# jordi-adell/mcarray

Measured on AMD Instinct MI355X. Metric: STFT frames/sec, 8-mic GCC-PHAT + SRP-PHAT(361) + delay-and-sum beamform @48kHz/1024-pt, higher is better.
Workload: dtype f32 (SRP operands adaptive); 1 GPU; BASELINE configs[2] geometry (8-mic ULA 0.04 m, 48 kHz, N=1024, hop 512, 361 angles, 1 source, no power floor), 8 arrays x 4096 frames per GPU per step; channel rows padded by 64 floats; arrays_per_gpu=8, frames_per_array=4096, srp_precision=adaptive, parallelism=arrays sharded over 1 GPU(s), all_gather of DOA bins+prob

## Files before the change

mcarray_amd/csrc/api.hip:

```cpp
#include "../../include/mcarray_hip.h"
#include "fft1024c.h"
#include "kernels.h"
#include "knobs.h"
#include "stage.h"

#include <chrono>
#include <cmath>
#include <cstdio>
#include <cstdlib>
#include <cstring>
#include <string>
#include <thread>
#include <vector>

using namespace mca;

namespace {

std::string g_create_error;

struct TimedEvent { int id; hipEvent_t a, b; };

}

// ... 1594 lines not shown

static bool steer_applies(const mca_hip_ctx *c)
{
    return !c->generic && !c->n512 && !c->n2048 && c->N == FFT_N && c->M == 8 && c->ula && c->S == 1 && !c->cfg.use_power_floor && c->merged &&
           (c->prec == MCA_HIP_SRP_ADAPTIVE || c->prec == MCA_HIP_SRP_FP16) && c->cfg.gcc_weighting != MCA_HIP_GCC_NONE;
}

static int steer_pass_frames(const mca_hip_ctx *c, int n_arrays, int n_frames)
{
    const long long cap = ws_max_bytes(c) / ((long long)n_arrays * STEER_ROW * (long long)sizeof(float2));
    return (int)std::max<long long>(1, std::min<long long>(n_frames, cap));
}

static void steer_policy_begin(mca_hip_ctx *c)
{
    const unsigned long long s = c->steer_seq + 1;
    if (!c->h_steer || c->steer_lost || s <= FB_LAG) return;
    const unsigned long long r = s - FB_LAG;
    if (r <= c->steer_seq_seen) return;
    const unsigned long long *slot = c->h_steer + 2 * ((r - 1) % FB_RING);
    const auto t0 = std::chrono::steady_clock::now();
    while (__atomic_load_n(&slot[1], __ATOMIC_ACQUIRE) != r) {
        if (std::chrono::duration_cast<std::chrono::milliseconds>(std::chrono::steady_clock::now() - t0).count() > FB_WAIT_MS) { c->steer_lost = true; c->steer_spec = true; return; }
        std::this_thread::yield();
    }
    c->steer_seq_seen = r;
    c->steer_spec = __atomic_load_n(&slot[0], __ATOMIC_RELAXED) * STEER_MISS_DEN <= c->steer_call_frames[(r - 1) % FB_RING] * STEER_MISS_NUM;
}

static int steer_prepare(mca_hip_ctx *c, int n_arrays, int n_frames)
{
    if (!c->d_steer_rows) {
        const size_t na = (size_t)c->cfg.max_arrays;
        HIP_TRY(c, hipMalloc((void **)&c->d_steer_rows, (size_t)(c->D + 1) * 4 * 64 * sizeof(float4)));
        HIP_TRY(c, hipMalloc((void **)&c->d_steer_q, (size_t)(c->D + 1) * c->M * 8 * sizeof(float2)));
        HIP_TRY(c, hipMalloc((void **)&c->d_steer_nyq, (size_t)(c->D + 1) * c->M * sizeof(float)));
        HIP_TRY(c, hipMalloc((void **)&c->d_steer_pred, na * sizeof(int)));
        HIP_TRY(c, hipMalloc((void **)&c->d_steer_miss, 3 * sizeof(unsigned long long)));
        if (hipHostMalloc((void **)&c->h_steer, FB_RING * 16, hipHostMallocDefault) == hipSuccess) std::memset(c->h_steer, 0, FB_RING * 16); else { c->h_steer = nullptr; (void)hipGetLastError(); }
        HIP_TRY(c, hipMalloc((void **)&c->d_steer_tail, 2 * na * FFT_H * sizeof(float)));
        HIP_TRY(c, hipMemset(c->d_steer_pred, 0xff, na * sizeof(int)));
        HIP_TRY(c, hipMemset(c->d_steer_miss, 0, 3 * sizeof(unsigned long long)));
        const double unit = (double)c->cfg.sample_rate / (double)FFT_N / 346.1;
        hipLaunchKernelGGL(k_steer_table, dim3(c->D + 1, 4), dim3(64), 0, nullptr, c->d_steer_rows, c->d_steer_q, c->d_steer_nyq, c->d_grid, c->d_micx, c->M, unit);
        HIP_TRY(c, hipGetLastError());
        HIP_TRY(c, hipDeviceSynchronize());
    }
    const size_t rows = (size_t)n_arrays * steer_pass_frames(c, n_arrays, n_frames);
    if (rows > c->steer_Y_rows) {
        HIP_TRY(c, hipDeviceSynchronize());
        if (c->d_steer_Y) (void)hipFree(c->d_steer_Y);
        c->d_steer_Y = nullptr; c->steer_Y_rows = 0;
        HIP_TRY(c, hipMalloc((void **)&c->d_steer_Y, rows * STEER_ROW * sizeof(float2)));
        c->steer_Y_rows = rows;
    }
    return MCA_HIP_OK;
}

static int steer_reserve(mca_hip_ctx *c, int n_arrays, int n_frames) { return steer_applies(c) ? steer_prepare(c, n_arrays, n_frames) : MCA_HIP_OK; }

static int steer_separate(mca_hip_ctx *c, const float *pcm, long long array_stride, long long mic_stride, int n_arrays, int n_frames,
                          const int *doa_bin, float *out_pcm, hipStream_t st)
{
    const size_t a0 = (size_t)c->a0;
    const int pf = steer_pass_frames(c, n_arrays, n_frames);
    const bool fused = c->steer_fused_now && pf == n_frames;
    const size_t smem = (size_t)(F1K_TWORDS + 4 * F1K_SCRATCH) * sizeof(float2);
    float *tails[2] = {c->d_steer_tail, c->d_steer_tail + (size_t)c->cfg.max_arrays * FFT_H};
    time_begin(c, MCA_HIP_K_BEAMFORM, st);
    int pass = 0;
    for (int f0 = 0; f0 < n_frames; f0 += pf, ++pass) {
        const int f1 = std::min(n_frames, f0 + pf), np = f1 - f0;
        const bool last = f1 == n_frames;
        SteerPatchArgs pa{};
        pa.pcm = pcm; pa.array_stride = array_stride; pa.mic_stride = mic_stride; pa.n_arrays = n_arrays; pa.n_frames = n_frames; pa.f0 = f0; pa.f1 = f1;
        pa.window = c->d_window; pa.doa_bin = doa_bin; pa.all = fused ? 0 : 1; pa.miss = c->d_steer_miss;
        pa.bf.rows = c->d_steer_rows; pa.bf.q = c->d_steer_q; pa.bf.nyq = c->d_steer_nyq; pa.bf.pred = c->d_steer_pred + a0; pa.bf.Y = c->d_steer_Y;
        pa.y_f0 = f0; pa.y_frames = fused ? n_frames : np;
        hipLaunchKernelGGL(k_steer_patch, dim3(std::min(STEER_PATCH_WGS, (np + 3) / 4)), dim3(256), smem, st, pa);
        SteerSynthArgs sy{};
        sy.Y = c->d_steer_Y; sy.n_frames = n_frames; sy.f0 = f0; sy.f1 = f1; sy.y_f0 = pa.y_f0; sy.y_frames = pa.y_frames;
        sy.ft = 16;
        while (sy.ft > 2 && (long long)n_arrays * ((np + sy.ft - 1) / sy.ft) < 1024) sy.ft >>= 1;
        sy.out = out_pcm;
        sy.tail_in = pass == 0 ? c->d_tail[c->tail_cur] + a0 * FFT_H : tails[(pass - 1) & 1];
        sy.tail_out = last ? c->d_tail[c->tail_cur ^ 1] + a0 * FFT_H : tails[pass & 1];
        sy.doa_bin = doa_bin; sy.pred_out = last ? c->d_steer_pred + a0 : nullptr;
        if (last && c->h_steer) { sy.report = c->h_steer + 2 * (c->steer_seq % FB_RING); sy.seq = c->steer_seq + 1; sy.miss_total = c->d_steer_miss; }
        const int runs = (np + sy.ft - 1) / sy.ft;
        hipLaunchKernelGGL(k_steer_synth, dim3((runs + 3) / 4, n_arrays), dim3(256), smem, st, sy);
    }
    time_end(c, st);
    HIP_TRY(c, hipGetLastError());
    c->steer_call_frames[c->steer_seq % FB_RING] = (unsigned long long)n_arrays * n_frames; ++c->steer_seq;
    c->steer_frames_total += (unsigned long long)n_arrays * n_frames;
    if (fused) ++c->steer_fused_calls;
    return MCA_HIP_OK;
}

static int separate_impl(mca_hip_ctx *c, const float *pcm, long long array_stride, long long mic_stride,
                         int n_arrays, int n_frames, const float *doa_rad, float *out_pcm, hipStream_t st, const int *doa_bin = nullptr)
{
    const size_t a0 = (size_t)c->a0;
    if (doa_bin && c->d_bftab && c->n2048 && (reinterpret_cast<uintptr_t>(out_pcm) & 7) == 0) {
        BeamformWaveArgs wa{};
        wa.pcm = pcm; wa.array_stride = array_stride; wa.mic_stride = mic_stride;
        wa.M = c->M; wa.n_pairs = c->M; wa.n_frames = n_frames; wa.S = c->S;
        wa.ft = 16;
        for (int ft = 2; ft <= 64; ++ft)
            if ((long long)n_arrays * c->S * ((n_frames + 4 * ft - 2) / (4 * ft - 1)) <= 2LL * c->n_cu) { wa.ft = ft; break; }
        wa.window = c->d_window; wa.doa_bin = doa_bin; wa.table = c->d_bftab; wa.out = out_pcm;
        wa.tail_in = c->d_tail[c->tail_cur] + a0 * c->S * c->H; wa.tail_out = c->d_tail[c->tail_cur ^ 1] + a0 * c->S * c->H;
        const int wgs = (n_frames + 4 * wa.ft - 2) / (4 * wa.ft - 1);
        const size_t smem_w = (size_t)(F1K_TWORDS + 4 * F1K_SCRATCH + 4 * 512) * sizeof(float2);
        time_begin(c, MCA_HIP_K_BEAMFORM, st);
        hipLaunchKernelGGL(k_beamform_wave_2048, dim3(wgs, n_arrays, c->S), dim3(256), smem_w, st, wa);
        time_end(c, st);
        HIP_TRY(c, hipGetLastError());
        return MCA_HIP_OK;
    }
    if (doa_bin && c->d_bftab && wave_beamformer_applies(c)) {
        BeamformWaveArgs wa{};
        wa.pcm = pcm; wa.array_stride = array_stride; wa.mic_stride = mic_stride;
        wa.M = c->M; wa.n_pairs = c->bf_pairs; wa.n_frames = n_frames; wa.S = c->S;
        wa.window = c->d_window; wa.doa_bin = doa_bin; wa.table = c->d_bftab; wa.out = out_pcm;
        wa.tail_in = c->d_tail[c->tail_cur] + a0 * c->S * c->H; wa.tail_out = c->d_tail[c->tail_cur ^ 1] + a0 * c->S * c->H;
        if (c->S >= 2 && c->M <= 8) {
            wa.ft = 16;
            while (wa.ft > 2 && (long long)n_arrays * ((n_frames + wa.ft - 1) / wa.ft) < 2048) wa.ft >>= 1;
            const int runs = (n_frames + wa.ft - 1) / wa.ft;
            const size_t smem_ms = (size_t)(F1K_TWORDS + 4 * F1K_SCRATCH) * sizeof(float2) + (size_t)4 * c->S * FFT_H * sizeof(float);
            const dim3 gms((runs + 3) / 4, n_arrays);
            time_begin(c, MCA_HIP_K_BEAMFORM, st);
#define BFMS(NPT)                                                                                                                   \
            do {                                                                                                                    \
                if (smem_ms > 64 * 1024) {                                                                                          \
                    HIP_TRY(c, hipFuncSetAttribute(reinterpret_cast<const void *>(&k_beamform_wave_ms<NPT, false>), hipFuncAttributeMaxDynamicSharedMemorySize, (int)smem_ms)); \
                    HIP_TRY(c, hipFuncSetAttribute(reinterpret_cast<const void *>(&k_beamform_wave_ms<NPT, true>), hipFuncAttributeMaxDynamicSharedMemorySize, (int)smem_ms));  \
                }                                                                                                                   \
                if (c->M & 1) hipLaunchKernelGGL((k_beamform_wave_ms<NPT, true>), gms, dim3(256), smem_ms, st, wa);                 \
                else hipLaunchKernelGGL((k_beamform_wave_ms<NPT, false>), gms, dim3(256), smem_ms, st, wa);                         \
            } while (0)
            if (c->bf_pairs == 1) {
                if (smem_ms > 64 * 1024) HIP_TRY(c, hipFuncSetAttribute(reinterpret_cast<const void *>(&k_beamform_wave_ms<1, false>), hipFuncAttributeMaxDynamicSharedMemorySize, (int)smem_ms));
                hipLaunchKernelGGL((k_beamform_wave_ms<1, false>), gms, dim3(256), smem_ms, st, wa);
            }
            else if (c->bf_pairs == 2) BFMS(2);
            else if (c->bf_pairs == 3) BFMS(3);
            else BFMS(4);
#undef BFMS
            time_end(c, st);
            HIP_TRY(c, hipGetLastError());
            return MCA_HIP_OK;
        }
        wa.ft = 2;
        while (wa.ft < 256 && (long long)n_arrays * c->S * ((n_frames + 4 * wa.ft - 2) / (4 * wa.ft - 1)) > 512) ++wa.ft;
        const int wgs = (n_frames + 4 * wa.ft - 2) / (4 * wa.ft - 1);
        const size_t smem = (size_t)(F1K_TWORDS + 4 * F1K_SCRATCH) * sizeof(float2) + 4 * FFT_H * sizeof(float);
        dim3 gb(wgs, n_arrays, c->S);
        if (c->S == 1 && (wgs & 1) == 0 && wa.ft >= 8 && (long long)wgs * n_arrays > (long long)c->n_cu * 3 / 2 && (long long)wgs * n_arrays <= 2LL * c->n_cu) {
            wa.skew = (3 * wa.ft + 8) / 16;
            if (wa.skew >= wa.ft) wa.skew = 0;
            else gb = dim3(n_arrays, wgs, c->S);
        }
        time_begin(c, MCA_HIP_K_BEAMFORM, st);
        if (c->M & 1) hipLaunchKernelGGL(k_beamform_wave<true>, gb, dim3(256), smem, st, wa);
// ... 956 lines not shown
```

mcarray_amd/csrc/fft1024c.h:

```cpp
#pragma once
#include "fft512.h"

namespace mca {

constexpr int F1K_ROW = 18;
constexpr int F1K_SCRATCH = 64 * F1K_ROW;
constexpr int F1K_TWORDS = 64 * F1K_ROW;

__device__ __forceinline__ void f1k_table_init(float2 *tab, int tid, int nthreads)
{
    for (int e = tid; e < 1024; e += nthreads) tab[(e >> 4) * F1K_ROW + (e & 15)] = twiddle(((e >> 4) * (e & 15)) & 1023, 1024, false);
}

__device__ __forceinline__ float2 csub_jb(float2 a, float2 b)
{
    v2f av = to_v2f(a), bv = to_v2f(b), r;
    asm("v_pk_fma_f32 %0, %2, 1.0, %1 op_sel:[1,0,0] op_sel_hi:[0,0,1] neg_hi:[1,0,0]" : "=v"(r) : "v"(av), "v"(bv));
    return from_v2f(r);
}
__device__ __forceinline__ float2 cadd_jb(float2 a, float2 b)
{
    v2f av = to_v2f(a), bv = to_v2f(b), r;
    asm("v_pk_fma_f32 %0, %2, 1.0, %1 op_sel:[1,0,0] op_sel_hi:[0,0,1] neg_lo:[1,0,0]" : "=v"(r) : "v"(av), "v"(bv));
    return from_v2f(r);
}
__device__ __forceinline__ float2 cscale(float2 a, float s)
{
    v2f av = to_v2f(a), sv = {s, s}, r;
    asm("v_pk_mul_f32 %0, %1, %2" : "=v"(r) : "v"(av), "v"(sv));
    return from_v2f(r);
}
__device__ __forceinline__ float2 cmul_mj(float2 a)
{
    v2f av = to_v2f(a), one = {1.f, 1.f}, r;
    asm("v_pk_mul_f32 %0, %1, %2 op_sel:[1,0] op_sel_hi:[0,1] neg_hi:[1,0]" : "=v"(r) : "v"(av), "v"(one));
    return from_v2f(r);
}
__device__ __forceinline__ float2 cmul_pj(float2 a)
{
    v2f av = to_v2f(a), one = {1.f, 1.f}, r;
    asm("v_pk_mul_f32 %0, %1, %2 op_sel:[1,0] op_sel_hi:[0,1] neg_lo:[1,0]" : "=v"(r) : "v"(av), "v"(one));
    return from_v2f(r);
}

template <bool INV>
__device__ __forceinline__ void bfly4(float2 &a0, float2 &a1, float2 &a2, float2 &a3)
{
    const float2 t0 = cadd(a0, a2), t1 = csub(a0, a2), t2 = cadd(a1, a3), t3 = csub(a1, a3);
    a0 = cadd(t0, t2);
    a2 = csub(t0, t2);
    if (!INV) { a1 = csub_jb(t1, t3); a3 = cadd_jb(t1, t3); }
    else { a1 = cadd_jb(t1, t3); a3 = csub_jb(t1, t3); }
}

__device__ __forceinline__ constexpr int dr16(int p) { return (p >> 2) + 4 * (p & 3); }

template <bool INV>
__device__ __forceinline__ void fft16(float2 (&v)[16])
{
    constexpr float R = 0.70710678118654752440f, C1 = 0.92387953251128675613f, S1 = 0.38268343236508977173f;
#pragma unroll
    for (int j = 0; j < 4; ++j) bfly4<INV>(v[j], v[j + 4], v[j + 8], v[j + 12]);
    const float2 w1 = make_float2(C1, -S1), w3 = make_float2(S1, -C1), w9 = make_float2(-C1, S1);
    if (!INV) {
        v[5] = cmul(v[5], w1);  v[9] = cscale(csub_jb(v[9], v[9]), R);   v[13] = cmul(v[13], w3);
        v[6] = cscale(csub_jb(v[6], v[6]), R);  v[10] = cmul_mj(v[10]);   v[14] = cscale(cadd_jb(v[14], v[14]), -R);
        v[7] = cmul(v[7], w3);  v[11] = cscale(cadd_jb(v[11], v[11]), -R); v[15] = cmul(v[15], w9);
    } else {
        v[5] = cmulc(v[5], w1); v[9] = cscale(cadd_jb(v[9], v[9]), R);   v[13] = cmulc(v[13], w3);
        v[6] = cscale(cadd_jb(v[6], v[6]), R);  v[10] = cmul_pj(v[10]);   v[14] = cscale(csub_jb(v[14], v[14]), -R);
        v[7] = cmulc(v[7], w3); v[11] = cscale(csub_jb(v[11], v[11]), -R); v[15] = cmulc(v[15], w9);
    }
#pragma unroll
    for (int q = 0; q < 4; ++q) bfly4<INV>(v[4 * q], v[4 * q + 1], v[4 * q + 2], v[4 * q + 3]);
}

__device__ __forceinline__ void lds_read16_b128(float2 (&v)[16], const float2 *p)
{
    typedef float v4f __attribute__((ext_vector_type(4)));
    v4f a[8];
    asm volatile(
        "ds_read_b128 %0, %8\n\tds_read_b128 %1, %8 offset:16\n\tds_read_b128 %2, %8 offset:32\n\tds_read_b128 %3, %8 offset:48\n\t"
        "ds_read_b128 %4, %8 offset:64\n\tds_read_b128 %5, %8 offset:80\n\tds_read_b128 %6, %8 offset:96\n\tds_read_b128 %7, %8 offset:112\n\t"
        "s_waitcnt lgkmcnt(0)"
        : "=&v"(a[0]), "=&v"(a[1]), "=&v"(a[2]), "=&v"(a[3]), "=&v"(a[4]), "=&v"(a[5]), "=&v"(a[6]), "=&v"(a[7])
        : "v"((unsigned)(uintptr_t)p)
        : "memory");
#pragma unroll
    for (int i = 0; i < 8; ++i) { v[2 * i] = make_float2(a[i].x, a[i].y); v[2 * i + 1] = make_float2(a[i].z, a[i].w); }
}

__device__ __forceinline__ void swap_rows32(float &a, float &b)
{
    const auto r = __builtin_amdgcn_permlane32_swap(__float_as_uint(a), __float_as_uint(b), false, false);
    a = __uint_as_float(r[0]); b = __uint_as_float(r[1]);
}
__device__ __forceinline__ void swap_rows16(float &a, float &b)
{
    const auto r = __builtin_amdgcn_permlane16_swap(__float_as_uint(a), __float_as_uint(b), false, false);
    a = __uint_as_float(r[0]); b = __uint_as_float(r[1]);
}
__device__ __forceinline__ void transpose_rows4(float2 &x0, float2 &x1, float2 &x2, float2 &x3)
{
    swap_rows32(x0.x, x2.x); swap_rows32(x0.y, x2.y); swap_rows32(x1.x, x3.x); swap_rows32(x1.y, x3.y);
    swap_rows16(x0.x, x1.x); swap_rows16(x0.y, x1.y); swap_rows16(x2.x, x3.x); swap_rows16(x2.y, x3.y);
}

struct F1kNoMid { __device__ __forceinline__ void operator()() const {} };

struct F1kLane {
    float2 wb[4];
    float2 t1[16];
    __device__ __forceinline__ void init(int lane)
    {
#pragma unroll
        for (int q = 1; q < 4; ++q) wb[q] = twiddle(((lane & 15) * q) & 63, 64, false);
    }
    __device__ __forceinline__ void load_t1(const float2 *tab, int lane)
    {
#pragma unroll
        for (int q = 0; q < 16; ++q) t1[q] = tab[lane * 18 + q];
    }
};

template <bool INV, int OPT = 3, typename Mid = F1kNoMid>
__device__ __forceinline__ void fft1024c(float2 (&v)[16], float2 *buf, int lane, const float2 *tab, const F1kLane &lc, Mid mid = Mid(), int row = -1)
{
    constexpr bool SCHED = OPT & 2, T1REG = OPT & 4;
    float2 tw[16];
    if (!T1REG) {
        lds_read16_b128(tw, tab + lane * F1K_ROW);
        if (SCHED) __builtin_amdgcn_sched_barrier(0);
    }
    fft16<INV>(v);
#pragma unroll
    for (int p = 1; p < 16; ++p) {
        const float2 w = T1REG ? lc.t1[dr16(p)] : tw[dr16(p)];
        v[p] = INV ? cmulc(v[p], w) : cmul(v[p], w);
    }
#pragma unroll
    for (int q = 0; q < 4; ++q) transpose_rows4(v[4 * q], v[4 * q + 1], v[4 * q + 2], v[4 * q + 3]);
#pragma unroll
    for (int q = 0; q < 4; ++q) bfly4<INV>(v[4 * q], v[4 * q + 1], v[4 * q + 2], v[4 * q + 3]);
    float2 *wr = buf + (lane >> 4) * (4 * F1K_ROW) + (lane & 15);
#pragma unroll
    for (int q = 0; q < 4; ++q)
#pragma unroll
        for (int kb = 0; kb < 4; ++kb) {
            if (kb != 0) v[4 * q + kb] = INV ? cmulc(v[4 * q + kb], lc.wb[kb]) : cmul(v[4 * q + kb], lc.wb[kb]);
            wr[(q + 16 * kb) * F1K_ROW] = v[4 * q + kb];
        }
    wave_lds_fence();
    mid();
    if (SCHED) __builtin_amdgcn_sched_barrier(0);
    lds_read16_b128(v, buf + (row < 0 ? lane : row) * F1K_ROW);
    wave_lds_fence();
    fft16<INV>(v);
}

}
```

mcarray_amd/csrc/kernels_wave.hip:

```cpp
#include <type_traits>

#include "fft1024c.h"
#include "mca_internal.h"
#include "cand_unit.h"
#include "phat_pairs.h"
#include "pair_balance.h"
#include "steer.h"

namespace mca {

__global__ __launch_bounds__(256) void k_bf_table(float2 *tab, const float *grid, const double *mic_x, int M, int n_pairs, double unit)
{
    const int d = blockIdx.x, pr = blockIdx.y;
    const double doa = d == 0 ? 0.0 : (double)grid[d - 1];
    const double cd = cos(doa + 1.57079632679489661923);
    const double sc = 1.0 / ((double)M * 1024.0);
    float2 *row = tab + ((long long)d * n_pairs + pr) * 1024;
    for (int k = threadIdx.x; k < 1024; k += 256) {
        const int kap = k <= 512 ? k : k - 1024;
        double pa[2] = {0.0, 0.0}, pb[2] = {0.0, 0.0};
        for (int e = 0; e < 2; ++e) {
            const int c = 2 * pr + e;
            if (c >= M) continue;
            double turns = (double)kap * (unit * mic_x[c] * cd);
// ... 539 lines not shown
                for (int s = 0; s < 8; ++s) {
                    if constexpr (ULA) {
                        float2 r[MT], out[NOUT];
#pragma unroll
                        for (int m = 0; m < MT; ++m) r[m] = Xh[m][s];
                        pair_products<MT, ULA>(r, out);
#pragma unroll
                        for (int g = 0; g < NOUT; ++g) store_a_wave<PL2>(arow, voff, g * KG + 64 * s, out[g], p.Kp);
                    } else {
                        int pi = 0;
#pragma unroll
                        for (int i = 0; i < MT; ++i)
#pragma unroll
                            for (int j = i + 1; j < MT; ++j) { store_a_wave<PL2>(arow, voff, pi * KG + 64 * s, cmulc(Xh[i][s], Xh[j][s]), p.Kp); ++pi; }
                    }
                }
            }
            if (POWER) {
                const float pacc = wave_sum64(ptime.x + ptime.y);
                if (lane == 0) p.power[(long long)a * p.total_frames + p.frame0 + f] = pacc / (float)FFT_N / (float)MT;
            }
        }
        wave_lds_fence();
        if (!MERGE && lane < f_end - f_begin) {
            float2 xn[MT], out[NOUT];
#pragma unroll
            for (int pr = 0; pr < NP; ++pr) {
                const float2 n = nyq[lane * NP + pr];
                float pw;
                xn[2 * pr] = whiten4<NOPHAT>(make_float2(2.f * n.x, 0.f), pw);
                xn[2 * pr + 1] = whiten4<NOPHAT>(make_float2(2.f * n.y, 0.f), pw);
            }
            OutT *arow = reinterpret_cast<OutT *>(p.A) + (row_base + f_begin + lane) * (long long)p.a_row_elems;
            pair_products<MT, ULA>(xn, out);
#pragma unroll
            for (int g = 0; g < NOUT; ++g) store_a_wave<PL2>(arow, 0u, g * KG + FFT_H, out[g], p.Kp);
        }
        }
        wave_lds_fence();
        if constexpr (CAND) {
            static_assert(!CAND || PL2, "the candidate contraction reads the two-plane rows of the list mode");
            {
                __syncthreads();
                cand_unit<4>(p.cand, li - p.list0, e_unit, reinterpret_cast<unsigned char *>(wbase), tid);
            }
        }
    }
}

__global__ __launch_bounds__(64) void k_steer_table(float4 *rows, float2 *q, float *nyq, const float *grid, const double *mic_x, int M, double unit)
{
    const int d = blockIdx.x, pr = blockIdx.y, lane = threadIdx.x, lam = lane <= 32 ? lane : 96 - lane;
    const double doa = d == 0 ? 0.0 : (double)grid[d - 1];
    const double cd = cos(doa + 1.57079632679489661923);
    const double sc = 1.0 / ((double)M * 1024.0);
    auto phasor = [&](int c, int k, double &cs, double &sn) {
        double turns = (double)k * (unit * mic_x[c] * cd);
        turns -= rint(turns);
        sincospi(2.0 * turns, &sn, &cs);
    };
    double ca, sa, cb, sb;
    phasor(2 * pr, lam, ca, sa); phasor(2 * pr + 1, lam, cb, sb);
    rows[((long long)d * gridDim.y + pr) * 64 + lane] = make_float4((float)(ca * sc), (float)(sa * sc), (float)(cb * sc), (float)(sb * sc));
    if (lane < 16) {
        const int c = 2 * pr + (lane >> 3), s = lane & 7;
        double cs, sn;
        phasor(c, 64 * s, cs, sn);
        q[((long long)d * M + c) * 8 + s] = make_float2((float)cs, (float)sn);
    }
    if (lane < 2) {
        double cs, sn;
        phasor(2 * pr + lane, 512, cs, sn);
        nyq[d * M + 2 * pr + lane] = (float)(cs * sc);
    }
}

__global__ __launch_bounds__(256, 2) void k_steer_patch(SteerPatchArgs p)
{
    constexpr int NP = 4, MT = 8;
    extern __shared__ __attribute__((aligned(16))) unsigned char smem_raw[];
    float2 *tab = reinterpret_cast<float2 *>(smem_raw);
    const int tid = threadIdx.x, lane = tid & 63, wave = __builtin_amdgcn_readfirstlane(tid >> 6);
    float2 *buf = tab + F1K_TWORDS + wave * F1K_SCRATCH;
    const int npass = p.f1 - p.f0, stride = 4 * (int)gridDim.x;
    int work = p.all;
    if (!work) {
        for (int a = 0; a < p.n_arrays; ++a) {
            const int pred = p.bf.pred[a];
            for (int fo = (int)blockIdx.x * 4 + wave + stride * lane; fo < npass; fo += stride * 64)
                work |= p.doa_bin[(long long)a * p.n_frames + p.f0 + fo] != pred;
        }
    }
    if (!__syncthreads_or(work)) return;
    f1k_table_init(tab, tid, 256);
    F1kLane lc;
    lc.init(lane);
    __syncthreads();
    const int lam = lane <= 32 ? lane : 96 - lane;
    const bool self = (lane & 31) == 0;
    v2f win[8];
#pragma unroll
    for (int i = 0; i < 8; ++i) { win[i].x = p.window[lane + 128 * i]; win[i].y = p.window[lane + 128 * i + 64]; }
    for (int a = 0; a < p.n_arrays; ++a) {
        const int pred = __builtin_amdgcn_readfirstlane(p.bf.pred[a]);
        const bool every = p.all != 0;
        int missed = 0;
        for (int fo = (int)blockIdx.x * 4 + wave; fo < npass; fo += stride) {
            const int f = p.f0 + fo;
            const int bin = __builtin_amdgcn_readfirstlane(p.doa_bin[(long long)a * p.n_frames + f]);
            if (bin != pred) ++missed;
            else if (!every) continue;
            const float4 *srow = p.bf.rows + (long long)(bin + 1) * (NP * 64);
            const float2 *qrow = p.bf.q + (long long)(bin + 1) * (MT * 8);
            const float *base = p.pcm + (long long)a * p.array_stride + (long long)f * FFT_H;
            float2 *yrow = p.bf.Y + ((long long)a * p.y_frames + f - p.y_f0) * STEER_ROW;
            float xa[16], xb[16];
            auto load_pair = [&](int pr) {
                const float *pa = base + (long long)(2 * pr) * p.mic_stride, *pb = pa + p.mic_stride;
#pragma unroll
                for (int i = 0; i < 16; ++i) { xa[i] = pa[(unsigned)lane + 64 * i]; xb[i] = pb[(unsigned)lane + 64 * i]; }
            };
            load_pair(0);
            float2 Y[8], zn[NP];
#pragma unroll
            for (int pr = 0; pr < NP; ++pr) {
                float2 z[16];
                float4 B;
#pragma unroll
                for (int i = 0; i < 8; ++i) { z[2 * i] = win_lo(xa[2 * i], xb[2 * i], win[i]); z[2 * i + 1] = win_hi(xa[2 * i + 1], xb[2 * i + 1], win[i]); }
                float ma = max3abs(z[0].x, z[1].x, z[2].x), mb = max3abs(z[0].y, z[1].y, z[2].y);
#pragma unroll
                for (int i = 3; i < 15; i += 2) { ma = max3abs(ma, z[i].x, z[i + 1].x); mb = max3abs(mb, z[i].y, z[i + 1].y); }
                ma = max2abs(ma, z[15].x); mb = max2abs(mb, z[15].y);
                const PairBalance pb = pair_balance(ma, mb);
                if (pb.scaled()) {
                    const float sa = pb.sa(), sb = pb.sb();
#pragma unroll
                    for (int i = 0; i < 16; ++i) z[i] = make_float2(z[i].x * sa, z[i].y * sb);
                }
                fft1024c<false, 3>(z, buf, lane, tab, lc, [&]() {
                    B = (srow + pr * 64)[(unsigned)lane];
                    if (pr < NP - 1) load_pair(pr + 1);
                }, lam);
                const float un_a = pb.un_a(), un_b = pb.un_b();
                zn[pr] = make_float2(z[dr16(8)].x * un_a, z[dr16(8)].y * un_b);
                const float4 Bu = steer_base(B, un_a, un_b);
                if (lane == 0) {
                    float2 t[16];
#pragma unroll
                    for (int j = 0; j < 16; ++j) t[j] = z[dr16(j)];
#pragma unroll
                    for (int j = 8; j < 16; ++j) z[dr16(j < 12 ? j + 4 : j - 4)] = t[(j + 1) & 15];
                } else if (self) {
#pragma unroll
                    for (int j = 8; j < 12; ++j) { const float2 t = z[dr16(j)]; z[dr16(j)] = z[dr16(j + 4)]; z[dr16(j + 4)] = t; }
                } else {
#pragma unroll
                    for (int j = 8; j < 12; ++j) {
                        float2 &u = z[dr16(j)], &w = z[dr16(j + 4)];
                        swap_rows32(u.x, w.x); swap_rows32(w.x, u.x);
                        swap_rows32(u.y, w.y); swap_rows32(w.y, u.y);
                    }
                }
#pragma unroll
                for (int s = 0; s < 8; ++s) {
                    const float2 zk = z[dr16(s)], zm = z[dr16(15 - s < 12 ? 15 - s + 4 : 15 - s - 4)];
                    const float2 a2 = make_float2(zk.x + zm.x, zk.y - zm.y);
                    const float2 b2 = make_float2(zk.y + zm.y, zm.x - zk.x);
                    const float2 y = pr == 0 ? make_float2(0.f, 0.f) : Y[s];
                    if (s == 0) Y[s] = steer_mac<true>(y, a2, b2, Bu, a2, b2);
                    else Y[s] = steer_mac<false>(y, a2, b2, Bu, qrow[(2 * pr) * 8 + s], qrow[(2 * pr + 1) * 8 + s]);
                }
                wave_lds_fence();
            }
#pragma unroll
            for (int s = 0; s < 8; ++s) yrow[(unsigned)lam + 64 * s] = s == 0 ? steer_dc(Y[s], lane) : Y[s];
            if (lane == 0) yrow[FFT_H] = make_float2(steer_nyquist<NP>(zn, p.bf.nyq + (bin + 1) * MT), 0.f);
        }
        if (missed && lane == 0) { atomicAdd(p.miss, (unsigned long long)missed); if (pred >= 0) atomicAdd(p.miss + 1, (unsigned long long)missed); }
    }
}

__global__ __launch_bounds__(256) void k_steer_synth(SteerSynthArgs p)
{
    extern __shared__ __attribute__((aligned(16))) unsigned char smem_raw[];
    float2 *tab = reinterpret_cast<float2 *>(smem_raw);
    const int tid = threadIdx.x, lane = tid & 63, wave = __builtin_amdgcn_readfirstlane(tid >> 6);
    float2 *buf = tab + F1K_TWORDS + wave * F1K_SCRATCH;
    f1k_table_init(tab, tid, 256);
    F1kLane lc;
    lc.init(lane);
    __syncthreads();
    const int a = blockIdx.y;
    if (p.pred_out && blockIdx.x == 0 && tid == 0) p.pred_out[a] = p.doa_bin[(long long)a * p.n_frames + p.n_frames - 1];
    if (p.report && blockIdx.x == 0 && a == 0 && tid == 0) {
        const unsigned long long tot = p.miss_total[1];
        p.report[0] = tot - p.miss_total[2];
        p.miss_total[2] = tot;
        __hip_atomic_store(&p.report[1], p.seq, __ATOMIC_RELEASE, __HIP_MEMORY_SCOPE_SYSTEM);
    }
    const int t0 = p.f0 + ((int)blockIdx.x * 4 + wave) * p.ft, t1 = min(t0 + p.ft, p.f1);
    if (t0 >= t1) return;
    const float2 *Yb = p.Y + ((long long)a * p.y_frames - p.y_f0) * STEER_ROW;
    float *ob = p.out + (long long)a * p.n_frames * FFT_H;
    float carry[8];
    if (t0 == p.f0) {
#pragma unroll
        for (int i = 0; i < 8; ++i) carry[i] = p.tail_in[(long long)a * FFT_H + lane + 64 * i];
    }
    int t = t0 > p.f0 ? t0 - 1 : t0;
    float2 yv[8], nv[8];
    float yn, nn = 0.f;
#pragma unroll
    for (int i = 0; i < 8; ++i) yv[i] = Yb[(long long)t * STEER_ROW + (unsigned)lane + 64 * i];
    yn = Yb[(long long)t * STEER_ROW + FFT_H].x;
    for (; t < t1; ++t) {
        float2 y[16];
        steer_inverse(y, yv, yn, buf, lane, tab, lc, [&]() {
            if (t + 1 < t1) {
#pragma unroll
                for (int i = 0; i < 8; ++i) nv[i] = Yb[(long long)(t + 1) * STEER_ROW + (unsigned)lane + 64 * i];
                nn = Yb[(long long)(t + 1) * STEER_ROW + FFT_H].x;
            }
        });
        if (t >= t0) {
#pragma unroll
            for (int i = 0; i < 8; ++i) ob[(long long)t * FFT_H + (unsigned)lane + 64 * i] = carry[i] + y[dr16(i)].x;
        }
#pragma unroll
        for (int i = 0; i < 8; ++i) { carry[i] = y[dr16(i + 8)].x; yv[i] = nv[i]; }
        yn = nn;
    }
    if (t1 == p.f1) {
#pragma unroll
        for (int i = 0; i < 8; ++i) p.tail_out[(long long)a * FFT_H + lane + 64 * i] = carry[i];
    }
}

typedef _Float16 h2 __attribute__((ext_vector_type(2)));
__device__ __forceinline__ h2 rot_j_conj(h2 b)
{
    h2 r;
    const unsigned c = 0x3C00BC00u;
    asm("v_pk_mul_f16 %0, %1, %2 op_sel:[1,0] op_sel_hi:[0,1]" : "=v"(r) : "v"(b), "v"(c));
    return r;
}

template <bool POWER>
__global__ __launch_bounds__(256, 2) void k_stft_phat_wave16(StftPhatArgs p)
{
    constexpr int MT = 16, NP = 8;
    extern __shared__ __attribute__((aligned(16))) unsigned char smem_raw[];
    float2 *tab = reinterpret_cast<float2 *>(smem_raw);
    const int tid = threadIdx.x, lane = tid & 63, wave = __builtin_amdgcn_readfirstlane(tid >> 6);
    float2 *buf = tab + F1K_TWORDS + wave * F1K_SCRATCH;
    float *wtab = reinterpret_cast<float *>(tab + F1K_TWORDS + 4 * F1K_SCRATCH);
    const int fpa = p.fpb + p.skew;
    float2 *nyq = reinterpret_cast<float2 *>(wtab + 1024) + wave * (fpa * NP);
    float2 *nref = reinterpret_cast<float2 *>(wtab + 1024) + 4 * (fpa * NP) + wave * (fpa * NP);
    float *dcbad = reinterpret_cast<float *>(reinterpret_cast<float2 *>(wtab + 1024) + 8 * (fpa * NP)) + wave * fpa;
    constexpr float UNSURE = 1e-10f;
    for (int e = tid; e < 1024; e += 256) wtab[(e & 63) * 16 + (e >> 6)] = p.window[e];
    f1k_table_init(tab, tid, 256);
    F1kLane lc;
    lc.init(lane);
    __syncthreads();
    const int lam = lane <= 32 ? lane : 96 - lane;
    const unsigned voff = (unsigned)lam * 4u;
    const bool self = (lane & 31) == 0;
    const float4 *wq = reinterpret_cast<const float4 *>(wtab + lane * 16);

    const int a = p.skew ? blockIdx.x : blockIdx.y;
    int f_begin = ((int)blockIdx.x * 4 + wave) * p.fpb, f_end = min(f_begin + p.fpb, p.n_frames);
    if (p.skew) {
        const int g = blockIdx.y, half = gridDim.y >> 1, hi = p.fpb + p.skew, lo = p.fpb - p.skew;
        if (g < half) { f_begin = (g * 4 + wave) * hi; f_end = f_begin + hi; }
        else { f_begin = half * 4 * hi + ((g - half) * 4 + wave) * lo; f_end = f_begin + lo; }
    }
    if (f_begin >= f_end) return;
    const long long row_base = (long long)a * p.n_frames;
    const float *base = p.pcm + (long long)a * p.array_stride + lane;
    float xa[16], xb[16];
    auto load_pair = [&](int f, int pr) {
        const float *pa = base + (long long)(2 * pr) * p.mic_stride + (long long)(p.frame0 + f) * FFT_H;
        const float *pb = pa + p.mic_stride;
#pragma unroll
        for (int i = 0; i < 16; ++i) { xa[i] = pa[64 * i]; xb[i] = pb[64 * i]; }
    };
    const int nfr = f_end - f_begin;
    const int rot = (int)((unsigned)(5 * a + 3 * ((int)blockIdx.x * 4 + wave)) % (unsigned)nfr);
    auto frame_of = [&](int i) { const int j = i + rot; return f_begin + (j >= nfr ? j - nfr : j); };
    load_pair(frame_of(0), 0);
    for (int fi = 0; fi < nfr; ++fi) {
        const int f = frame_of(fi);
        h2 Xh[MT][8];
        v2f ptime = {0.f, 0.f};
        bool dc_unsure = false;
#pragma unroll
        for (int pr = 0; pr < NP; ++pr) {
            float2 z[16];
#pragma unroll
            for (int i4 = 0; i4 < 4; ++i4) {
                const float4 w4 = wq[i4];
                const v2f w01 = {w4.x, w4.y}, w23 = {w4.z, w4.w};
                z[4 * i4] = win_lo(xa[4 * i4], xb[4 * i4], w01); z[4 * i4 + 1] = win_hi(xa[4 * i4 + 1], xb[4 * i4 + 1], w01);
                z[4 * i4 + 2] = win_lo(xa[4 * i4 + 2], xb[4 * i4 + 2], w23); z[4 * i4 + 3] = win_hi(xa[4 * i4 + 3], xb[4 * i4 + 3], w23);
            }
            float ref_a = 0.f, ref_b = 0.f;
            if (POWER || p.unsure) {
                v2f pz = {0.f, 0.f};
#pragma unroll
                for (int i = 0; i < 16; ++i) { const v2f zv = to_v2f(z[i]); asm("v_pk_fma_f32 %0, %1, %1, %0" : "+v"(pz) : "v"(zv)); }
                if (POWER) { ptime.x += pz.x; ptime.y += pz.y; }
                if (p.unsure) { ref_a = 4.f * wave_sum64(pz.x); ref_b = 4.f * wave_sum64(pz.y); }
// ... 127 lines not shown
```

mcarray_amd/csrc/mca_internal.h:

```cpp
#pragma once
#include <hip/hip_runtime.h>

#define MCA_MAX_SOURCES 4
#define MCA_MAX_MICS 16

namespace mca {

constexpr int MK_NB = 4;
constexpr int MK_WARM = 8;
constexpr int BF_NB = 4;
constexpr int GCC2_DOAWARM = 64;
constexpr int SCAN_WARM = 96;
constexpr int KG = 513;
#ifndef MCA_SCAN_CHUNK
#define MCA_SCAN_CHUNK 32
#endif
#ifndef MCA_SCAN_SUB
#define MCA_SCAN_SUB 32
#endif
constexpr int SCAN_CHUNK = MCA_SCAN_CHUNK;
constexpr int SCAN_SUB = MCA_SCAN_SUB;
#ifndef MCA_SCAN_LD
#define MCA_SCAN_LD 8
#endif
constexpr int SCAN_LD = MCA_SCAN_LD;
#ifndef MCA_REPAIR_WARM
#define MCA_REPAIR_WARM 16
#endif
constexpr int REPAIR_WARM = MCA_REPAIR_WARM;
constexpr int REPAIR_GROUP = 4;
constexpr int HIST_FRAMES = REPAIR_WARM, HIST_UNITS = HIST_FRAMES / REPAIR_GROUP, HIST_SAMPLES = (HIST_FRAMES + 1) * 512;
static_assert(HIST_FRAMES % REPAIR_GROUP == 0, "history = whole repair units");

constexpr int CAND_WORDS_MAX = 20;
struct CandArgs {
    const void *A;
    const void *B;
    int Kp, Dp, a_row_elems;
    const int *list; const int *n_list; int list0, pass_rows;
    unsigned *umask; int umask_words;
    int *need;
    int groups_per_array, n_frames;
    float *C; int c_planes; long long c_plane_stride;
    float *hist_C; int hist_base;
};

constexpr int STEER_QWORDS = 8 * 7;
constexpr int STEER_LDS_ROWS = 13;
constexpr int STEER_Y_ZN = 8, STEER_Y_BASE = 11;
constexpr int STEER_MISS_NUM = 1, STEER_MISS_DEN = 3;
constexpr int STEER_ROW = 520;
struct SteerArgs {
    const float4 *rows;
    const float2 *q;
    const float *nyq;
    const int *pred;
    float2 *Y;
};
constexpr int STEER_PATCH_WGS = 512;
struct SteerPatchArgs {
    const float *pcm; long long array_stride, mic_stride;
    int n_arrays, n_frames;
    int f0, f1;
    const float *window;
    const int *doa_bin;
    SteerArgs bf;
    int y_f0, y_frames;
    int all;
    unsigned long long *miss;
};
struct SteerSynthArgs {
    const float2 *Y; int n_frames, f0, f1, ft, y_f0, y_frames;
    float *out;
    const float *tail_in; float *tail_out;
    const int *doa_bin; int *pred_out;
    unsigned long long *report; unsigned long long seq; unsigned long long *miss_total;
};

struct StftPhatArgs {
    const float *pcm;
    long long array_stride, mic_stride;
    int M, n_frames, frame0, fpb;
    const float *window;
    void *A;
    int Kp;
    int a_row_elems;
    int a_planes;
    float *power;
    int total_frames;
    int N, logH, kg, ula;
    const float2 *tw;
    const int *list; const int *n_list; int list0, list_cap, groups_per_array;
    float *hist_out; const float *hist_in; int hist_base;
    const unsigned short *mrank; int n_merged;
    int no_phat;
    int skew;
    unsigned char *dead;
    unsigned char *unsure;
    int cand_on; CandArgs cand;
    SteerArgs bf;
};

__device__ __forceinline__ void store_a(float *row, const StftPhatArgs &, int cidx, float2 v)
{
    reinterpret_cast<float2 *>(row)[cidx] = v;
}

typedef _Float16 half2_t __attribute__((ext_vector_type(2)));

typedef float float2_t __attribute__((ext_vector_type(2)));

__device__ __forceinline__ void store_a(_Float16 *row, const StftPhatArgs &p, int cidx, float2 v)
{
    const float2_t vv = {v.x, v.y};
    const half2_t hi = __builtin_convertvector(vv, half2_t);
    reinterpret_cast<half2_t *>(row)[cidx] = hi;
    if (p.a_planes == 2) {
        const float2_t back = __builtin_convertvector(hi, float2_t);
        const half2_t lo = __builtin_convertvector(vv - back, half2_t);
        reinterpret_cast<half2_t *>(row + p.Kp)[cidx] = lo;
    }
}

struct GemmArgs {
    const void *A;
    const void *B;
    float *C;
    int rows;
    int chunk_frames, total_frames, frame0;
    int Kp, Dp, a_row_elems;
    long long c_plane_elems;
    const void *Bt;
    const int *n_list; int list0;
    int repair_ksplit;
    int repair_items;
    float *part; int *nvoiced; int D, n_chunks;
    long long part_plane_stride;
    float scan_w[32];
};

struct ScanPickArgs {
    const float *C;
    int c_planes; long long c_plane_stride;
    int n_frames, Dp, D, P, S, chunk, n_chunks;
    float mu, one_minus_mu;
    float inv_norm;
    const float *state_in;
    float *state_out;
    float *part;
    int part_planes; long long part_plane_stride;
    int *nvoiced;
    float *e_start;
    const unsigned char *voiced;
    const float *grid;
    int *doa_bin; float *doa_rad; float *prob; float *energy;
// ... 378 lines not shown
```

mcarray_amd/csrc/steer.h:

```cpp
#pragma once
#include "fft1024c.h"

namespace mca {

__device__ __forceinline__ float4 steer_base(float4 B, float un_a, float un_b)
{
    const float2 a = cscale(make_float2(B.x, B.y), un_a), b = cscale(make_float2(B.z, B.w), un_b);
    return make_float4(a.x, a.y, b.x, b.y);
}
template <bool FIRST>
__device__ __forceinline__ float2 steer_mac(float2 y, float2 a2, float2 b2, float4 B, float2 qa, float2 qb)
{
    if (!FIRST) { a2 = cmul(a2, qa); b2 = cmul(b2, qb); }
    y = cmac(y, a2, make_float2(B.x, B.y));
    return cmac(y, b2, make_float2(B.z, B.w));
}
__device__ __forceinline__ float2 steer_dc(float2 y0, int lane) { return cscale(y0, lane == 0 ? 0.5f : 1.f); }

template <int NP>
__device__ __forceinline__ float steer_nyquist(const float2 (&zn)[NP], const float *pn)
{
    float yn = 0.f;
#pragma unroll
    for (int pr = 0; pr < NP; ++pr) yn = fmaf(zn[pr].y, pn[2 * pr + 1], fmaf(zn[pr].x, pn[2 * pr], yn));
    return yn;
}

template <typename Mid = F1kNoMid>
__device__ __forceinline__ void steer_inverse(float2 (&y)[16], const float2 (&yv)[8], float yn, float2 *buf, int lane, const float2 *tab, const F1kLane &lc, Mid mid = Mid())
{
#pragma unroll
    for (int i = 0; i < 8; ++i) { y[i] = yv[i]; y[i + 8] = make_float2(0.f, 0.f); }
    fft1024c<true, 3>(y, buf, lane, tab, lc, mid);
    const float sn = (lane & 1) ? -yn : yn;
#pragma unroll
    for (int i = 0; i < 16; ++i) y[i].x += sn;
}

}
```

Baseline: 57.47 million frames/s.

## Restructure steer patch/synth: slot-ballot scheduling, warmup handoff, and half-zero inverse FFT

Steer patch now flattens (array, frame) pairs into slots, evaluates DOA misses via wave ballots, and processes only missed slots. It also prefetches the first PCM pair and window before table init, and accumulates miss counters per block. Steer synth adds an LDS handoff between waves so non-lead waves skip recomputing the previous frame's inverse FFT for overlap-add, and the inverse FFT uses a specialized first radix-16 stage that exploits the zero upper half. This adds a block barrier and more complex indexing, with a risk of ordering bugs in the handoff.

```diff
diff --git a/mcarray_amd/csrc/api.hip b/mcarray_amd/csrc/api.hip
--- a/mcarray_amd/csrc/api.hip
+++ b/mcarray_amd/csrc/api.hip
@@ -1700,6 +1700,7 @@
         sy.Y = c->d_steer_Y; sy.n_frames = n_frames; sy.f0 = f0; sy.f1 = f1; sy.y_f0 = pa.y_f0; sy.y_frames = pa.y_frames;
         sy.ft = 16;
         while (sy.ft > 2 && (long long)n_arrays * ((np + sy.ft - 1) / sy.ft) < 1024) sy.ft >>= 1;
+        sy.handoff = sy.ft == 16;
         sy.out = out_pcm;
         sy.tail_in = pass == 0 ? c->d_tail[c->tail_cur] + a0 * FFT_H : tails[(pass - 1) & 1];
         sy.tail_out = last ? c->d_tail[c->tail_cur ^ 1] + a0 * FFT_H : tails[pass & 1];
diff --git a/mcarray_amd/csrc/fft1024c.h b/mcarray_amd/csrc/fft1024c.h
--- a/mcarray_amd/csrc/fft1024c.h
+++ b/mcarray_amd/csrc/fft1024c.h
@@ -75,6 +75,23 @@
     for (int q = 0; q < 4; ++q) bfly4<INV>(v[4 * q], v[4 * q + 1], v[4 * q + 2], v[4 * q + 3]);
 }
 
+__device__ __forceinline__ void fft16_inv_lo8(float2 (&v)[16])
+{
+    constexpr float R = 0.70710678118654752440f, C1 = 0.92387953251128675613f, S1 = 0.38268343236508977173f;
+#pragma unroll
+    for (int j = 0; j < 4; ++j) {
+        const float2 a0 = v[j], a1 = v[j + 4];
+        v[j] = cadd(a0, a1); v[j + 8] = csub(a0, a1);
+        v[j + 4] = cadd_jb(a0, a1); v[j + 12] = csub_jb(a0, a1);
+    }
+    const float2 w1 = make_float2(C1, -S1), w3 = make_float2(S1, -C1), w9 = make_float2(-C1, S1);
+    v[5] = cmulc(v[5], w1); v[9] = cscale(cadd_jb(v[9], v[9]), R);   v[13] = cmulc(v[13], w3);
+    v[6] = cscale(cadd_jb(v[6], v[6]), R);  v[10] = cmul_pj(v[10]);   v[14] = cscale(csub_jb(v[14], v[14]), -R);
+    v[7] = cmulc(v[7], w3); v[11] = cscale(csub_jb(v[11], v[11]), -R); v[15] = cmulc(v[15], w9);
+#pragma unroll
+    for (int q = 0; q < 4; ++q) bfly4<true>(v[4 * q], v[4 * q + 1], v[4 * q + 2], v[4 * q + 3]);
+}
+
 __device__ __forceinline__ void lds_read16_b128(float2 (&v)[16], const float2 *p)
 {
     typedef float v4f __attribute__((ext_vector_type(4)));
@@ -158,4 +175,33 @@
     fft16<INV>(v);
 }
 
-}
+template <typename Mid = F1kNoMid>
+__device__ __forceinline__ void fft1024c_inv_lo8(float2 (&v)[16], float2 *buf, int lane, const float2 *tab, const F1kLane &lc, Mid mid = Mid())
+{
+    float2 tw[16];
+    lds_read16_b128(tw, tab + lane * F1K_ROW);
+    __builtin_amdgcn_sched_barrier(0);
+    fft16_inv_lo8(v);
+#pragma unroll
+    for (int p = 1; p < 16; ++p) v[p] = cmulc(v[p], tw[dr16(p)]);
+#pragma unroll
+    for (int q = 0; q < 4; ++q) transpose_rows4(v[4 * q], v[4 * q + 1], v[4 * q + 2], v[4 * q + 3]);
+#pragma unroll
+    for (int q = 0; q < 4; ++q) bfly4<true>(v[4 * q], v[4 * q + 1], v[4 * q + 2], v[4 * q + 3]);
+    float2 *wr = buf + (lane >> 4) * (4 * F1K_ROW) + (lane & 15);
+#pragma unroll
+    for (int q = 0; q < 4; ++q)
+#pragma unroll
+        for (int kb = 0; kb < 4; ++kb) {
+            if (kb != 0) v[4 * q + kb] = cmulc(v[4 * q + kb], lc.wb[kb]);
+            wr[(q + 16 * kb) * F1K_ROW] = v[4 * q + kb];
+        }
+    wave_lds_fence();
+    mid();
+    __builtin_amdgcn_sched_barrier(0);
+    lds_read16_b128(v, buf + lane * F1K_ROW);
+    wave_lds_fence();
+    fft16<true>(v);
+}
+
+}
diff --git a/mcarray_amd/csrc/kernels_wave.hip b/mcarray_amd/csrc/kernels_wave.hip
--- a/mcarray_amd/csrc/kernels_wave.hip
+++ b/mcarray_amd/csrc/kernels_wave.hip
@@ -645,45 +645,73 @@
     float2 *tab = reinterpret_cast<float2 *>(smem_raw);
     const int tid = threadIdx.x, lane = tid & 63, wave = __builtin_amdgcn_readfirstlane(tid >> 6);
     float2 *buf = tab + F1K_TWORDS + wave * F1K_SCRATCH;
-    const int npass = p.f1 - p.f0, stride = 4 * (int)gridDim.x;
-    int work = p.all;
-    if (!work) {
-        for (int a = 0; a < p.n_arrays; ++a) {
-            const int pred = p.bf.pred[a];
-            for (int fo = (int)blockIdx.x * 4 + wave + stride * lane; fo < npass; fo += stride * 64)
-                work |= p.doa_bin[(long long)a * p.n_frames + p.f0 + fo] != pred;
-        }
-    }
-    if (!__syncthreads_or(work)) return;
+    const int npass = p.f1 - p.f0, stride = 4 * (int)gridDim.x, first = (int)blockIdx.x * 4 + wave;
+    const int nown = first < npass ? (npass - 1 - first) / stride + 1 : 0, nslot = nown * p.n_arrays;
+    const unsigned ndiv = (unsigned)max(nown, 1);
+    struct Slot { int pred, bin; bool in; };
+    auto ask = [&](int s0) {
+        const unsigned s = (unsigned)(s0 + lane), q = s / ndiv;
+        Slot r;
+        r.in = (int)s < nslot;
+        const unsigned a = r.in ? q : 0u;
+        r.pred = p.bf.pred[a];
+        r.bin = p.doa_bin[r.in ? (long long)a * p.n_frames + p.f0 + first + stride * (int)(s - a * ndiv) : 0];
+        return r;
+    };
+    int missed = 0, guarded = 0;
+    auto judge = [&](const Slot &r) {
+        const bool miss = r.in && r.bin != r.pred;
+        const unsigned long long m = __ballot(miss);
+        missed += __popcll(m);
+        guarded += __popcll(__ballot(miss && r.pred >= 0));
+        return p.all ? __ballot(r.in) : m;
+    };
+    const Slot r0 = ask(0), r1 = ask(64);
+    const unsigned long long todo0 = judge(r0), todo1 = judge(r1);
+    unsigned long long later = 0;
+    for (int s0 = 128; s0 < nslot; s0 += 64) later |= judge(ask(s0));
+    if (!__syncthreads_or((todo0 | todo1 | later) != 0)) return;
+    if (missed && lane == 0) { atomicAdd(p.miss, (unsigned long long)missed); if (guarded) atomicAdd(p.miss + 1, (unsigned long long)guarded); }
+    float xa[16], xb[16];
+    auto load_pair = [&](const float *base, int pr) {
+        const float *pa = base + (long long)(2 * pr) * p.mic_stride, *pb = pa + p.mic_stride;
+#pragma unroll
+        for (int i = 0; i < 16; ++i) { xa[i] = pa[(unsigned)lane + 64 * i]; xb[i] = pb[(unsigned)lane + 64 * i]; }
+    };
+    auto slot_base = [&](int s, int &a, int &f) {
+        a = s / (int)ndiv; f = p.f0 + first + stride * (s - a * (int)ndiv);
+        return p.pcm + (long long)a * p.array_stride + (long long)f * FFT_H;
+    };
+    bool primed = (todo0 | todo1) != 0;
+    v2f win[8];
+    if (primed) {
+        int a, f;
+        load_pair(slot_base(todo0 ? __builtin_ctzll(todo0) : 64 + __builtin_ctzll(todo1), a, f), 0);
+    }
+#pragma unroll
+    for (int i = 0; i < 8; ++i) { win[i].x = p.window[lane + 128 * i]; win[i].y = p.window[lane + 128 * i + 64]; }
     f1k_table_init(tab, tid, 256);
     F1kLane lc;
     lc.init(lane);
     __syncthreads();
     const int lam = lane <= 32 ? lane : 96 - lane;
     const bool self = (lane & 31) == 0;
-    v2f win[8];
-#pragma unroll
-    for (int i = 0; i < 8; ++i) { win[i].x = p.window[lane + 128 * i]; win[i].y = p.window[lane + 128 * i + 64]; }
-    for (int a = 0; a < p.n_arrays; ++a) {
-        const int pred = __builtin_amdgcn_readfirstlane(p.bf.pred[a]);
-        const bool every = p.all != 0;
-        int missed = 0;
-        for (int fo = (int)blockIdx.x * 4 + wave; fo < npass; fo += stride) {
-            const int f = p.f0 + fo;
-            const int bin = __builtin_amdgcn_readfirstlane(p.doa_bin[(long long)a * p.n_frames + f]);
-            if (bin != pred) ++missed;
-            else if (!every) continue;
+    for (int s0 = 0; s0 < nslot; s0 += 64) {
+        unsigned long long todo;
+        int binv;
+        if (s0 == 0) { todo = todo0; binv = r0.bin; }
+        else if (s0 == 64) { todo = todo1; binv = r1.bin; }
+        else { const Slot r = ask(s0); todo = p.all ? __ballot(r.in) : __ballot(r.in && r.bin != r.pred); binv = r.bin; }
+        for (; todo; todo &= todo - 1) {
+            const int l = __builtin_ctzll(todo);
+            const int bin = __builtin_amdgcn_readlane(binv, l);
+            int a, f;
+            const float *base = slot_base(s0 + l, a, f);
             const float4 *srow = p.bf.rows + (long long)(bin + 1) * (NP * 64);
             const float2 *qrow = p.bf.q + (long long)(bin + 1) * (MT * 8);
-            const float *base = p.pcm + (long long)a * p.array_stride + (long long)f * FFT_H;
             float2 *yrow = p.bf.Y + ((long long)a * p.y_frames + f - p.y_f0) * STEER_ROW;
-            float xa[16], xb[16];
-            auto load_pair = [&](int pr) {
-                const float *pa = base + (long long)(2 * pr) * p.mic_stride, *pb = pa + p.mic_stride;
-#pragma unroll
-                for (int i = 0; i < 16; ++i) { xa[i] = pa[(unsigned)lane + 64 * i]; xb[i] = pb[(unsigned)lane + 64 * i]; }
-            };
-            load_pair(0);
+            if (!primed) load_pair(base, 0);
+            primed = false;
             float2 Y[8], zn[NP];
 #pragma unroll
             for (int pr = 0; pr < NP; ++pr) {
@@ -703,7 +731,7 @@
                 }
                 fft1024c<false, 3>(z, buf, lane, tab, lc, [&]() {
                     B = (srow + pr * 64)[(unsigned)lane];
-                    if (pr < NP - 1) load_pair(pr + 1);
+                    if (pr < NP - 1) load_pair(base, pr + 1);
                 }, lam);
                 const float un_a = pb.un_a(), un_b = pb.un_b();
                 zn[pr] = make_float2(z[dr16(8)].x * un_a, z[dr16(8)].y * un_b);
@@ -740,7 +768,6 @@
             for (int s = 0; s < 8; ++s) yrow[(unsigned)lam + 64 * s] = s == 0 ? steer_dc(Y[s], lane) : Y[s];
             if (lane == 0) yrow[FFT_H] = make_float2(steer_nyquist<NP>(zn, p.bf.nyq + (bin + 1) * MT), 0.f);
         }
-        if (missed && lane == 0) { atomicAdd(p.miss, (unsigned long long)missed); if (pred >= 0) atomicAdd(p.miss + 1, (unsigned long long)missed); }
     }
 }
 
@@ -750,11 +777,28 @@
     float2 *tab = reinterpret_cast<float2 *>(smem_raw);
     const int tid = threadIdx.x, lane = tid & 63, wave = __builtin_amdgcn_readfirstlane(tid >> 6);
     float2 *buf = tab + F1K_TWORDS + wave * F1K_SCRATCH;
+    const int a = blockIdx.y;
+    const int t0 = p.f0 + ((int)blockIdx.x * 4 + wave) * p.ft, t1 = min(t0 + p.ft, p.f1);
+    const bool active = t0 < t1, lead = wave == 0 || !p.handoff;
+    const float2 *Yb = p.Y + ((long long)a * p.y_frames - p.y_f0) * STEER_ROW;
+    float *ob = p.out + (long long)a * p.n_frames * FFT_H;
+    float carry[8], head[8];
+    int t = lead && t0 > p.f0 ? t0 - 1 : t0;
+    float2 yv[8], nv[8];
+    float yn = 0.f, nn = 0.f;
+    if (active) {
+        if (t0 == p.f0) {
+#pragma unroll
+            for (int i = 0; i < 8; ++i) carry[i] = p.tail_in[(long long)a * FFT_H + lane + 64 * i];
+        }
+#pragma unroll
+        for (int i = 0; i < 8; ++i) yv[i] = Yb[(long long)t * STEER_ROW + (unsigned)lane + 64 * i];
+        yn = Yb[(long long)t * STEER_ROW + FFT_H].x;
+    }
     f1k_table_init(tab, tid, 256);
     F1kLane lc;
     lc.init(lane);
     __syncthreads();
-    const int a = blockIdx.y;
     if (p.pred_out && blockIdx.x == 0 && tid == 0) p.pred_out[a] = p.doa_bin[(long long)a * p.n_frames + p.n_frames - 1];
     if (p.report && blockIdx.x == 0 && a == 0 && tid == 0) {
         const unsigned long long tot = p.miss_total[1];
@@ -762,37 +806,37 @@
         p.miss_total[2] = tot;
         __hip_atomic_store(&p.report[1], p.seq, __ATOMIC_RELEASE, __HIP_MEMORY_SCOPE_SYSTEM);
     }
-    const int t0 = p.f0 + ((int)blockIdx.x * 4 + wave) * p.ft, t1 = min(t0 + p.ft, p.f1);
-    if (t0 >= t1) return;
-    const float2 *Yb = p.Y + ((long long)a * p.y_frames - p.y_f0) * STEER_ROW;
-    float *ob = p.out + (long long)a * p.n_frames * FFT_H;
-    float carry[8];
-    if (t0 == p.f0) {
-#pragma unroll
-        for (int i = 0; i < 8; ++i) carry[i] = p.tail_in[(long long)a * FFT_H + lane + 64 * i];
-    }
-    int t = t0 > p.f0 ? t0 - 1 : t0;
-    float2 yv[8], nv[8];
-    float yn, nn = 0.f;
-#pragma unroll
-    for (int i = 0; i < 8; ++i) yv[i] = Yb[(long long)t * STEER_ROW + (unsigned)lane + 64 * i];
-    yn = Yb[(long long)t * STEER_ROW + FFT_H].x;
-    for (; t < t1; ++t) {
-        float2 y[16];
-        steer_inverse(y, yv, yn, buf, lane, tab, lc, [&]() {
-            if (t + 1 < t1) {
-#pragma unroll
-                for (int i = 0; i < 8; ++i) nv[i] = Yb[(long long)(t + 1) * STEER_ROW + (unsigned)lane + 64 * i];
-                nn = Yb[(long long)(t + 1) * STEER_ROW + FFT_H].x;
-            }
-        });
-        if (t >= t0) {
-#pragma unroll
-            for (int i = 0; i < 8; ++i) ob[(long long)t * FFT_H + (unsigned)lane + 64 * i] = carry[i] + y[dr16(i)].x;
-        }
-#pragma unroll
-        for (int i = 0; i < 8; ++i) { carry[i] = y[dr16(i + 8)].x; yv[i] = nv[i]; }
-        yn = nn;
+    if (active) {
+        for (; t < t1; ++t) {
+            float2 y[16];
+            steer_inverse(y, yv, yn, buf, lane, tab, lc, [&]() {
+                if (t + 1 < t1) {
+#pragma unroll
+                    for (int i = 0; i < 8; ++i) nv[i] = Yb[(long long)(t + 1) * STEER_ROW + (unsigned)lane + 64 * i];
+                    nn = Yb[(long long)(t + 1) * STEER_ROW + FFT_H].x;
+                }
+            });
+            if (!lead && t == t0) {
+#pragma unroll
+                for (int i = 0; i < 8; ++i) head[i] = y[dr16(i)].x;
+            } else if (t >= t0) {
+#pragma unroll
+                for (int i = 0; i < 8; ++i) ob[(long long)t * FFT_H + (unsigned)lane + 64 * i] = carry[i] + y[dr16(i)].x;
+            }
+#pragma unroll
+            for (int i = 0; i < 8; ++i) { carry[i] = y[dr16(i + 8)].x; yv[i] = nv[i]; }
+            yn = nn;
+        }
+        if (p.handoff) {
+#pragma unroll
+            for (int i = 0; i < 8; ++i) reinterpret_cast<float *>(buf)[lane + 64 * i] = carry[i];
+        }
+    }
+    if (p.handoff) __syncthreads();
+    if (!active) return;
+    if (!lead) {
+#pragma unroll
+        for (int i = 0; i < 8; ++i) ob[(long long)t0 * FFT_H + (unsigned)lane + 64 * i] = reinterpret_cast<const float *>(buf - F1K_SCRATCH)[lane + 64 * i] + head[i];
     }
     if (t1 == p.f1) {
 #pragma unroll
diff --git a/mcarray_amd/csrc/mca_internal.h b/mcarray_amd/csrc/mca_internal.h
--- a/mcarray_amd/csrc/mca_internal.h
+++ b/mcarray_amd/csrc/mca_internal.h
@@ -71,6 +71,7 @@
 };
 struct SteerSynthArgs {
     const float2 *Y; int n_frames, f0, f1, ft, y_f0, y_frames;
+    int handoff;
     float *out;
     const float *tail_in; float *tail_out;
     const int *doa_bin; int *pred_out;
diff --git a/mcarray_amd/csrc/steer.h b/mcarray_amd/csrc/steer.h
--- a/mcarray_amd/csrc/steer.h
+++ b/mcarray_amd/csrc/steer.h
@@ -30,8 +30,8 @@
 __device__ __forceinline__ void steer_inverse(float2 (&y)[16], const float2 (&yv)[8], float yn, float2 *buf, int lane, const float2 *tab, const F1kLane &lc, Mid mid = Mid())
 {
 #pragma unroll
-    for (int i = 0; i < 8; ++i) { y[i] = yv[i]; y[i + 8] = make_float2(0.f, 0.f); }
-    fft1024c<true, 3>(y, buf, lane, tab, lc, mid);
+    for (int i = 0; i < 8; ++i) y[i] = yv[i];
+    fft1024c_inv_lo8(y, buf, lane, tab, lc, mid);
     const float sn = (lane & 1) ? -yn : yn;
 #pragma unroll
     for (int i = 0; i < 16; ++i) y[i].x += sn;
```

Result: no change. 58.00 million frames/s, median of 6 (+0.9%).
